# SCoulY/MuSCLe

Hardware: AMD Instinct MI355X
Metric: images/sec (whole node), MCL EfficientNet-B7 448x448 bs=32/GPU (higher is better)
Workload: dtype f32; 1 GPU; train_mcl.py loop body, step-A (epoch-4 gates: focal+softmargin+pairwise+ER+IMC, one backward, one Adam step), MuSCLe(efficientnet-b7, last_pooling=False, 21 classes), random-init weights; per_gpu_batch=32, global_batch=32, image=448x448, parallelism=single, optimizer=Adam(lr=1e-4, wd=5e-5) fused, launch=eager, weight-gradient GEMMs on a second stream

## Files before the change

### include/muscle_hip.h

```cpp
#ifndef MUSCLE_HIP_H
#define MUSCLE_HIP_H

#ifdef __cplusplus
extern "C" {
#endif

int mx_version(void);
int mx_abi_hash(void);
const char* mx_last_error(void);


int mx_pw_fwd_parts(int M, int N, int K);
int mx_pw_fwd(const float* A, int a_mode, const float* a_scale, const float* a_shift, const float* a_gate,
              int rows_per_sample, const float* W, float* C, int M, int K, int N, int lda, int ldc,
              const float* bias, const float* residual, int relu, float* stats, void* stream);

int mx_set_gemm_mode(int mode);
int mx_get_gemm_mode(void);
int mx_set_wgrad_kernel(int kernel, int groups);
int mx_get_wgrad_kernel(void);
int mx_gemm_uses_split(int kind, int M, int N, int K);

long mx_pw_planes_bytes(int N, int K);
int mx_pw_planes_tiles(int N, int K);
int mx_pw_planes_batch(const long* table, int n, int total_tiles, void* stream);
int mx_pw_fwd_uses_planes(int M, int K, int N);
int mx_pw_fwd_planes(const float* A, const void* Wplanes, float* C, int M, int K, int N, int lda, int ldc,
                     const float* bias, const float* residual, int relu, float* stats, void* stream);

int mx_transpose(const float* src, float* dst, int rows, int cols, void* stream);
int mx_transpose_batch(const long* table, int n, int total_tiles, void* stream);

int mx_pw_dgrad(const float* G, const float* W, float* dX, int M, int K, int N, int ldg, int ldx,
                const float* residual, void* stream);

int mx_pw_dgrad_bnbwd(const float* G, const float* X, const float* coef, const float* Wt, float* dX, float* dZ, int M, int K, int N,
                      int ldg, int ldx, const float* residual, void* stream);

int mx_pw_fwd_act_uses_planes(int M, int K, int N);
int mx_pw_fwd_planes_act(const float* A, const float* scale, const float* shift, const float* gate, int rows_per_sample,
                         const void* Wplanes, float* C, int M, int K, int N, int lda, int ldc, float* stats, void* stream);

int mx_pw_dgrad_bnbwd_planes(const float* G, const float* X, const float* coef, const void* WtPlanes, float* dX, int M, int K, int N,
// ... 30 lines not shown
int mx_colreduce_parts(long rows, int C);
int mx_colstats(const float* X, long rows, int C, float* part, void* stream);

int mx_bn_finalize(const float* part, int P, int C, double count, const float* gamma, const float* beta, float* running_mean,
                   float* running_var, float momentum, float eps, int training, float* scale, float* shift,
                   float* mean, float* rstd, double* acc , void* stream);

int mx_fold_block(const float* We, const float* g0, const float* b0, const float* m0, const float* v0, float eps0,
                  const float* g1, const float* b1, const float* m1, const float* v1, float eps1,
                  const float* Wp, const float* g2, const float* b2, const float* m2, const float* v2, float eps2,
                  int Cin, int Cexp, int Cout, float* We_f, float* be, float* s1, float* t1, float* Wp_f, float* bp, void* stream);

int mx_bn_apply(const float* P, const float* scale, const float* shift, const float* row_scale, const float* residual,
                const float* gate, float* out, long rows, int C, int rows_per_sample, int act, void* stream);

int mx_bn_bwd_reduce(const float* G, const float* X, const float* row_scale, const float* gate, const float* gate_add,
                     const float* act_scale, const float* act_shift, long rows, int C, int rows_per_sample,
                     float* part, void* stream);

int mx_bn_bwd_finalize(const float* part, int P, int C, double count, const float* gamma, const float* mean, const float* rstd,
                       int training, float* dgamma, float* dbeta, float* c1, float* c2, float* c3, double* acc,
                       void* stream);

int mx_bn_bwd_apply(const float* G, const float* X, const float* row_scale, const float* gate, const float* gate_add,
                    const float* act_scale, const float* act_shift, const float* c1, const float* c2, const float* c3,
                    float* out, long rows, int C, int rows_per_sample, void* stream);

long mx_pool_ws(long rows, int C, int rows_per_sample, int planes);
int mx_pool_sum(const float* X, const float* G, const float* scale, const float* shift, int act, long rows, int C,
                int rows_per_sample, float* out, void* ws, long ws_bytes, void* stream);

int mx_se_bn1_pool(const float* dA, const float* X, const float* scale, const float* shift, long rows, int C, int rows_per_sample,
                   float* out5, void* ws, long ws_bytes, void* stream);
int mx_bn1_sums_finalize(const float* pooled5, const float* gate, const float* gh, const float* W1, float inv_hw, float* add,
                         int N, int C, int SQ, double count, const float* gamma, const float* mean, const float* rstd, int training,
                         float* dgamma, float* dbeta, float* c1, float* c2, float* c3, void* stream);


int mx_dwconv_fwd_parts(int N, int Ho, int Wo, int C, int S);
long mx_dwconv_fwd_ws(int N, int Ho, int Wo, int C, int S);
int mx_dwconv_fwd(const float* X, const float* scale, const float* shift, const float* W, float* Y, float* stats,
// ... 175 lines not shown
```

### muscle_amd/csrc/bn.hip

```cpp
#include "common.h"

struct ColGeom {
  int rows, C, c4;
  int tcols;
  int rpp;
  int rows_per_block;
  int rps;
};

static ColGeom col_geom(long rows, int C, int rps, long rows_limit ,
                        int groups = 1 , int planes = 1) {
  ColGeom g;
  g.rows = (int)rows; g.C = C; g.c4 = C / 4; g.rps = rps;
  {
    const int cand[] = {g.c4 <= 256 ? g.c4 : 256, 256, 192, 128, 96, 64, 48, 32};
    double best = -1.0;
    g.tcols = cand[0];
    for (int tc : cand) {
      if (tc > g.c4) continue;
      const double util = (double)g.c4 / (double)(cdiv(g.c4, tc) * tc) * (double)(256 / tc * tc) / 256.0;
      if (groups > 1 ? util > best - 1e-9 : util > best + 1e-9) { best = util; g.tcols = tc; }
    }
  }
  g.rpp = 256 / g.tcols;
// ... 482 lines not shown
  int dr, dc, dn, drem, c4n, rps;
  __device__ __forceinline__ RowWalk(long i0, long stride, int c4n_, int rps_) : c4n(c4n_), rps(rps_) {
    r = i0 / c4n; c4 = (int)(i0 - r * c4n);
    n = (int)(r / rps); rem = (int)(r - (long)n * rps);
    const long sr = stride / c4n;
    dr = (int)sr; dc = (int)(stride - sr * c4n);
    dn = dr / rps; drem = dr - dn * rps;
  }
  __device__ __forceinline__ void next() {
    c4 += dc; r += dr; n += dn; rem += drem;
    if (c4 >= c4n) { c4 -= c4n; ++r; ++rem; }
    if (rem >= rps) { rem -= rps; ++n; }
  }
};

__global__ __launch_bounds__(256) void bn_apply_kernel(const float* P, const float* sc, const float* sh, const float* rs,
                                                       const float* R, const float* gate, float* out, long total4, int C,
                                                       int rps, int act) {
  RowWalk w(blockIdx.x * 256L + threadIdx.x, (long)gridDim.x * 256, C / 4, rps);
  for (long i = blockIdx.x * 256L + threadIdx.x; i < total4; i += (long)gridDim.x * 256, w.next()) {
    const int c = w.c4 * 4;
    float4 v = ld4(P + i * 4);
    float4 a = ld4(sc + c), b = ld4(sh + c);
    v.x = a.x * v.x + b.x; v.y = a.y * v.y + b.y; v.z = a.z * v.z + b.z; v.w = a.w * v.w + b.w;
    if (act) { v.x = swishf_(v.x); v.y = swishf_(v.y); v.z = swishf_(v.z); v.w = swishf_(v.w); }
    if (gate) { float4 g = ld4(gate + (long)w.n * C + c); v.x *= g.x; v.y *= g.y; v.z *= g.z; v.w *= g.w; }
    if (rs) { float s = rs[w.n]; v.x *= s; v.y *= s; v.z *= s; v.w *= s; }
    if (R) { float4 q = ld4(R + i * 4); v.x += q.x; v.y += q.y; v.z += q.z; v.w += q.w; }
    st4(out + i * 4, v);
  }
}

__global__ __launch_bounds__(256) void bn_bwd_apply_kernel(GEff e, const float* c1, const float* c2, const float* c3,
                                                           float* out, long total4) {
  RowWalk w(blockIdx.x * 256L + threadIdx.x, (long)gridDim.x * 256, e.C / 4, e.rps);
  for (long i = blockIdx.x * 256L + threadIdx.x; i < total4; i += (long)gridDim.x * 256, w.next()) {
    const int c = w.c4 * 4;
    float4 g, x;
    e.get_n(w.r, w.n, c, g, x);
    float4 k1 = ld4(c1 + c), k2 = ld4(c2 + c), k3 = ld4(c3 + c);
    float4 o;
    o.x = k1.x * g.x + k2.x * x.x + k3.x; o.y = k1.y * g.y + k2.y * x.y + k3.y;
    o.z = k1.z * g.z + k2.z * x.z + k3.z; o.w = k1.w * g.w + k2.w * x.w + k3.w;
    st4(out + i * 4, o);
  }
}

static int grid_for(long total4) {
  static const long cap = getenv("MX_STREAM_BLOCKS") ? atol(getenv("MX_STREAM_BLOCKS")) : 4096;
  long b = (total4 + 255) / 256;
  return (int)(b < cap ? (b < 1 ? 1 : b) : cap);
}

struct FoldArgs {
  const float *We, *g0, *b0, *m0, *v0, *g1, *b1, *m1, *v1, *Wp, *g2, *b2, *m2, *v2;
  float eps0, eps1, eps2;
  int Cin, Cexp, Cout;
  float *We_f, *be, *s1, *t1, *Wp_f, *bp;
};
// ... 67 lines not shown
    MX_LAUNCH_CHECK();
    return MX_OK;
  }
  int slices = 0;
  if (training) slices = launch_parts_reduce(part, P, C, acc, (hipStream_t)stream);
  hipLaunchKernelGGL(bn_finalize_kernel, dim3(cdiv(C, 32)), dim3(256), 0, (hipStream_t)stream, acc, slices, C, count, gamma,
                     beta, running_mean, running_var, momentum, eps, training, scale, shift, mean, rstd);
  MX_LAUNCH_CHECK();
  return MX_OK;
}

int mx_bn_apply(const float* P, const float* scale, const float* shift, const float* row_scale, const float* residual,
                const float* gate, float* out, long rows, int C, int rows_per_sample, int act, void* stream) {
  MX_CHECK_ARG(P && scale && shift && out && rows > 0 && C % 4 == 0 && rows_per_sample > 0, "bn_apply: bad args");
  long total4 = rows * (C / 4);
  hipLaunchKernelGGL(bn_apply_kernel, dim3(grid_for(total4)), dim3(256), 0, (hipStream_t)stream, P, scale, shift,
                     row_scale, residual, gate, out, total4, C, rows_per_sample, act);
  MX_LAUNCH_CHECK();
  return MX_OK;
}

int mx_bn_bwd_reduce(const float* G, const float* X, const float* row_scale, const float* gate, const float* gate_add,
                     const float* act_scale, const float* act_shift, long rows, int C, int rows_per_sample,
                     float* part, void* stream) {
  MX_CHECK_ARG(G && X && part && rows > 0 && C % 4 == 0 && rows_per_sample > 0, "bn_bwd_reduce: bad args");
  MX_CHECK_ARG((gate == nullptr) == (gate_add == nullptr), "bn_bwd_reduce: gate and gate_add come together");
  MX_CHECK_ARG((act_scale == nullptr) == (act_shift == nullptr), "bn_bwd_reduce: act scale/shift come together");
  FBwdReduce f{GEff{G, X, row_scale, gate, gate_add, act_scale, act_shift, C, rows_per_sample}};
  launch_colreduce<FBwdReduce, 2, false, float>(f, rows, C, rows_per_sample, part, part, (hipStream_t)stream);
  MX_LAUNCH_CHECK();
  return MX_OK;
}
// ... 9 lines not shown
    return MX_OK;
  }
  const int slices = launch_parts_reduce(part, P, C, acc, (hipStream_t)stream);
  hipLaunchKernelGGL(bn_bwd_finalize_kernel, dim3(cdiv(C, 32)), dim3(256), 0, (hipStream_t)stream, acc, slices, C, count, gamma,
                     mean, rstd, training, dgamma, dbeta, c1, c2, c3);
  MX_LAUNCH_CHECK();
  return MX_OK;
}

int mx_bn_bwd_apply(const float* G, const float* X, const float* row_scale, const float* gate, const float* gate_add,
                    const float* act_scale, const float* act_shift, const float* c1, const float* c2, const float* c3,
                    float* out, long rows, int C, int rows_per_sample, void* stream) {
  MX_CHECK_ARG(G && X && out && c1 && c2 && c3 && rows > 0 && C % 4 == 0 && rows_per_sample > 0, "bn_bwd_apply: bad args");
  GEff e{G, X, row_scale, gate, gate_add, act_scale, act_shift, C, rows_per_sample};
  long total4 = rows * (C / 4);
  hipLaunchKernelGGL(bn_bwd_apply_kernel, dim3(grid_for(total4)), dim3(256), 0, (hipStream_t)stream, e, c1, c2, c3, out,
                     total4);
  MX_LAUNCH_CHECK();
  return MX_OK;
}

long mx_pool_ws(long rows, int C, int rows_per_sample, int planes) {
  if (rows <= 0 || C <= 0 || C % 4 || rows_per_sample <= 0 || rows % rows_per_sample || (planes != 1 && planes != 5)) return MX_EARG;
  return pool_ws_bytes(rows, C, rows_per_sample, planes);
}

int mx_se_bn1_pool(const float* dA, const float* X, const float* scale, const float* shift, long rows, int C, int rows_per_sample,
                   float* out5, void* ws, long ws_bytes, void* stream) {
  MX_CHECK_ARG(dA && X && scale && shift && out5 && rows > 0 && C % 4 == 0 && rows_per_sample > 0 && rows % rows_per_sample == 0,
               "se_bn1_pool: bad args");
  const int N = (int)(rows / rows_per_sample);
  dim3 grid;
// ... 41 lines not shown
```

### muscle_amd/csrc/common.h

```cpp
#pragma once
#include <hip/hip_runtime.h>
#include <stdint.h>

#define MX_OK 0
#define MX_EARG (-1)

extern "C" const char* mx_last_error(void);
void mx_set_error(const char* fmt, ...);

#define MX_CHECK_ARG(cond, ...)            \
  do {                                     \
    if (!(cond)) {                         \
      mx_set_error(__VA_ARGS__);           \
      return MX_EARG;                      \
    }                                      \
  } while (0)

#define MX_LAUNCH_CHECK()                                     \
  do {                                                        \
    hipError_t e__ = hipGetLastError();                       \
    if (e__ != hipSuccess) {                                  \
      mx_set_error("launch failed: %s", hipGetErrorString(e__)); \
      return (int)e__;                                        \
    }                                                         \
// ... 126 lines not shown
  for (int i = 1; i < 8; ++i) { s0 += sh[i * 32 + cl]; s1 += sh[256 + i * 32 + cl]; }
  bn_bwd_finalize_one(c, s0, s1, b.count, b.gamma, b.mean, b.rstd, b.training, b.dgamma, b.dbeta, b.c1, b.c2, b.c3);
}

__device__ __forceinline__ float4 ld4(const float* p) { return *reinterpret_cast<const float4*>(p); }
__device__ __forceinline__ void st4(float* p, float4 v) { *reinterpret_cast<float4*>(p) = v; }

struct MxOperand {
  const float* p;
  const float* c1;
  const float* c2;
  const float* rowp;
  int mode;
  int rps;
};
enum { MX_PLAIN = 0, MX_BNACT = 1, MX_AFFINE = 2, MX_BNBWD = 3 };

__device__ __forceinline__ float4 mx_apply(const MxOperand& o, float4 v, long r, int c, int cols) {
  if (o.mode == MX_PLAIN) return v;
  float4 a = ld4(o.c1 + c), b = ld4(o.c2 + c);
  v.x = a.x * v.x + b.x; v.y = a.y * v.y + b.y; v.z = a.z * v.z + b.z; v.w = a.w * v.w + b.w;
  if (o.mode == MX_AFFINE) return v;
  v.x = swishf_(v.x); v.y = swishf_(v.y); v.z = swishf_(v.z); v.w = swishf_(v.w);
  if (o.rowp) {
    float4 g = ld4(o.rowp + (r / o.rps) * (long)cols + c);
    v.x *= g.x; v.y *= g.y; v.z *= g.z; v.w *= g.w;
  }
  return v;
}
```

### muscle_amd/csrc/gemm.hip

```cpp
#include "common.h"
#include <type_traits>
#include <stdlib.h>

typedef float f32x16 __attribute__((ext_vector_type(16)));
typedef float f32x4 __attribute__((ext_vector_type(4)));

struct GemmArgs {
  MxOperand a, b;
  float* c;
  int M, N, K;
  int lda, ldb, ldc;
  long sa, sb, sc;
  const float* bias;
  const float* residual;
  int relu;
  float* stats;
  int ksplit;
  int xcd_nt;
  int mt, zt;
  unsigned long long* stamps;
  float* a_out;
  float* ws;
};

// ... 568 lines not shown
    for (int st = 0; st < 4; ++st)
#pragma unroll
      for (int i = 0; i < TM; ++i)
#pragma unroll
        for (int j = 0; j < TN; ++j)
          acc[i][j] = __builtin_amdgcn_mfma_f32_16x16x4f32(bv[j][st], av[i][st], acc[i][j], 0, 0, 0);
    __syncthreads();
  }
  MX_GEMM_STAMP(g, 2);
  nt_epilogue<WM, WN, TM, TN>(g, C, tile_m, m0, n0, acc, smem, tid);
  MX_GEMM_STAMP(g, 3);
}

typedef __bf16 bf16x8 __attribute__((ext_vector_type(8)));

static __device__ __forceinline__ void split3_pair(float x0, float x1, unsigned& h, unsigned& m, unsigned& l) {
  const unsigned u0 = __float_as_uint(x0) & 0xffff0000u, u1 = __float_as_uint(x1) & 0xffff0000u;
  const float r0 = x0 - __uint_as_float(u0), r1 = x1 - __uint_as_float(u1);
  const unsigned v0 = __float_as_uint(r0) & 0xffff0000u, v1 = __float_as_uint(r1) & 0xffff0000u;
  const float s0 = r0 - __uint_as_float(v0), s1 = r1 - __uint_as_float(v1);
  h = __builtin_amdgcn_perm(u1, u0, 0x07060302u);
  m = __builtin_amdgcn_perm(v1, v0, 0x07060302u);
  l = __builtin_amdgcn_perm(__float_as_uint(s1), __float_as_uint(s0), 0x07060302u);
}

template <int AMODE, int NJ>
__global__ __launch_bounds__(256, NJ == 4 ? 2 : 3) void gemm_nt_split_kernel(GemmArgs g) {
  constexpr int BM = 128, BN = 64 * NJ, WN = 2, WNC = 32 * NJ;
  constexpr int PA_ = 128 * 32, PB_ = BN * 32;
  constexpr int STAGE = 3 * PA_ + 3 * PB_;
  constexpr int PS = WNC + 4;
  constexpr int SMEM = (2 * STAGE > 4 * 32 * PS * 4 + 2 * 2 * BN * 4) ? 2 * STAGE : 4 * 32 * PS * 4 + 2 * 2 * BN * 4;
  __shared__ __attribute__((aligned(16))) unsigned char smem[SMEM];
  const int tid = threadIdx.x, lane = tid & 63, wave = tid >> 6;
  const int l31 = lane & 31, hf = lane >> 5;
  const int wm = wave / WN, wn = wave % WN;
  int tile_m = blockIdx.x, tile_n = blockIdx.y;
  if (g.xcd_nt > 0) {
    const int L = blockIdx.x, xcd = L & 7, j = L >> 3;
// ... 257 lines not shown
    const int chunk = blockIdx.x / per_chunk, L = blockIdx.x % per_chunk, xcd = L & 7, j = L >> 3;
    tile_n = chunk * g.xcd_nt + j % g.xcd_nt;
    tile_m = (j / g.xcd_nt) * 8 + xcd;
    if (tile_m >= g.mt || tile_n >= g.zt) return;
  }
  const int m0 = tile_m * BM, n0 = tile_n * BN;
  const long zb = blockIdx.z;
  const float* A = g.a.p + zb * g.sa;
  const unsigned char* WP = reinterpret_cast<const unsigned char*>(g.b.p);
  float* C = g.c + zb * g.sc;
  const int nk = (g.K + 31) >> 5;
  const bool ktail = (g.K & 31) != 0;
  const long npad64 = (long)g.ldb * 64;

  const float* ap[2];
#pragma unroll
  for (int i = 0; i < 2; ++i) {
    const int gr = min(m0 + 32 * wave + 16 * i + l15, g.M - 1);
    ap[i] = A + (long)gr * g.lda + 4 * q;
  }
  const unsigned char* wsrc[WPW];
  int wdst[WPW];
#pragma unroll
  for (int i = 0; i < WPW; ++i) {
    const int pw = wave + 4 * i, p = pw / (BN / 16), rp = pw % (BN / 16);
    wsrc[i] = WP + ((long)p * g.ldb + n0 + 16 * rp) * 64 + lane * 16;
    wdst[i] = p * W_PLANE + rp * 1024;
  }
  auto issue_w = [&](int kt) {
    unsigned char* st = smem + (kt & 1) * STAGE;
#pragma unroll
    for (int i = 0; i < WPW; ++i)
      if (WPIECES % 4 == 0 || wave + 4 * i < WPIECES) glds16(wsrc[i] + 3 * npad64 * kt, st + wdst[i]);
  };
  f32x4 raw[2][2];
  f32x4 rawx[(AMODE == MX_BNBWD || AMODE == MX_BNACT) ? 2 : 1][2], cf[AMODE == MX_BNBWD ? 3 : AMODE == MX_BNACT ? 2 : 1][2];
  const long xoff = AMODE == MX_BNBWD ? (g.a.rowp + zb * g.sa) - A : 0;
  const float* gp[AMODE == MX_BNACT ? 2 : 1];
  if (AMODE == MX_BNACT) {
#pragma unroll
    for (int i = 0; i < 2; ++i) {
      const int gr = min(m0 + 32 * wave + 16 * i + l15, g.M - 1);
      gp[AMODE == MX_BNACT ? i : 0] = g.a.rowp + (long)(gr / g.a.rps) * g.K + 4 * q;
    }
  }
  auto load_a = [&](int kt) {
    const bool half = AMODE != MX_BNBWD && ktail && kt == nk - 1;
#pragma unroll
    for (int i = 0; i < 2; ++i) {
      raw[i][0] = *reinterpret_cast<const f32x4*>(ap[i] + 32 * kt);
      raw[i][1] = half ? f32x4{0.f, 0.f, 0.f, 0.f} : *reinterpret_cast<const f32x4*>(ap[i] + 32 * kt + 16);
      if (AMODE == MX_BNBWD) {
        rawx[AMODE == MX_BNBWD ? i : 0][0] = *reinterpret_cast<const f32x4*>(ap[i] + xoff + 32 * kt);
        rawx[AMODE == MX_BNBWD ? i : 0][1] = *reinterpret_cast<const f32x4*>(ap[i] + xoff + 32 * kt + 16);
      }
      if (AMODE == MX_BNACT) {
        rawx[AMODE == MX_BNACT ? i : 0][0] = *reinterpret_cast<const f32x4*>(gp[AMODE == MX_BNACT ? i : 0] + 32 * kt);
        rawx[AMODE == MX_BNACT ? i : 0][1] = *reinterpret_cast<const f32x4*>(gp[AMODE == MX_BNACT ? i : 0] + 32 * kt + 16);
      }
    }
    if (AMODE == MX_BNACT) {
// ... 15 lines not shown
#pragma unroll
  for (int i = 0; i < 2; ++i)
#pragma unroll
    for (int j = 0; j < TN; ++j) acc[i][j] = f32x4{0.f, 0.f, 0.f, 0.f};
  const int woff = l15 * 64 + ((q ^ swz_w(l15)) << 4);

  MX_GEMM_STAMP(g, 0);
  issue_w(0);
  load_a(0);
  MX_GEMM_STAMP(g, 1);
  for (int kt = 0; kt < nk; ++kt) {
    asm volatile("s_waitcnt vmcnt(0)" ::: "memory");
    bf16x8 af[2][3];
#pragma unroll
    for (int i = 0; i < 2; ++i) {
      if (AMODE == MX_BNBWD) {
#pragma unroll
        for (int u = 0; u < 2; ++u)
#pragma unroll
          for (int e = 0; e < 4; ++e)
            raw[i][u][e] = cf[0][u][e] * raw[i][u][e] + (cf[AMODE == MX_BNBWD ? 1 : 0][u][e] * rawx[AMODE == MX_BNBWD ? i : 0][u][e] +
                                                         cf[AMODE == MX_BNBWD ? 2 : 0][u][e]);
      }
      if (AMODE == MX_BNACT) {
#pragma unroll
        for (int u = 0; u < 2; ++u)
#pragma unroll
          for (int e = 0; e < 4; ++e)
            raw[i][u][e] = swishf_(cf[0][u][e] * raw[i][u][e] + cf[AMODE == MX_BNACT ? 1 : 0][u][e]) * rawx[AMODE == MX_BNACT ? i : 0][u][e];
      }
// ... 80 lines not shown
static void launch_nt_split3_t(const GemmArgs& g, int batch, hipStream_t st) {
  constexpr int BN = 16 * TN;
  const int mt = cdiv(g.M, 128), nt = cdiv(g.N, BN);
  GemmArgs a = g;
  a.mt = mt;
  a.xcd_nt = 0;
  dim3 grid(mt, nt, batch);
  if (nt >= 2 && mt >= 64) {
    const int chunks = nt <= 16 ? 1 : cdiv(nt, g_split3_xcd_chunk);
    a.xcd_nt = cdiv(nt, chunks); a.zt = nt;
    grid = dim3(chunks * 8 * cdiv(mt, 8) * a.xcd_nt, 1, batch);
  }
  if (g.a.mode == MX_BNBWD) hipLaunchKernelGGL((gemm_nt_split3_kernel<TN, MX_BNBWD>), grid, dim3(256), 0, st, a);
  else if (g.a.mode == MX_BNACT) {
    if constexpr (TN <= 6) hipLaunchKernelGGL((gemm_nt_split3_kernel<TN, MX_BNACT>), grid, dim3(256), 0, st, a);
  } else hipLaunchKernelGGL((gemm_nt_split3_kernel<TN, MX_PLAIN>), grid, dim3(256), 0, st, a);
}

static int g_split_nj = getenv("MX_GEMM_SPLIT_NJ") ? atoi(getenv("MX_GEMM_SPLIT_NJ")) : 0;
static void launch_nt_split3(const GemmArgs& g, int batch, hipStream_t st) {
  auto cost = [&](int bn, double eff) {
    const double per_cu = (double)cdiv(g.M, 128) * cdiv(g.N, bn) * batch / 256.0;
    return (per_cu + 0.5) * bn / eff;
  };
  const long wide_tiles = (long)cdiv(g.M, 128) * cdiv(g.N, 128) * batch;
  int bn = 128;
  if (g_split_nj >= 16) bn = g_split_nj;
  else if (g_split_nj == 1 || (g_split_nj != 2 && wide_tiles <= 300)) bn = 64;
  else if (g_split_nj != 2) {
    const bool shortk = g.K <= 512;
    const double e64 = shortk ? 0.90 : 0.85, e80 = shortk ? 0.97 : 0.90, e96 = shortk ? 1.03 : 0.94, e112 = 0.97;
// ... 209 lines not shown
  hipLaunchKernelGGL(split_planes_kernel, dim3(total_tiles), dim3(256), 0, (hipStream_t)stream, table, n);
  MX_LAUNCH_CHECK();
  return MX_OK;
}

int mx_pw_fwd_uses_planes(int M, int K, int N) {
  static const int on = getenv("MX_SPLIT2") ? atoi(getenv("MX_SPLIT2")) : 1;
  static const int early = getenv("MX_SPLIT3_EARLY") ? atoi(getenv("MX_SPLIT3_EARLY")) : 1;
  static const int tail = getenv("MX_SPLIT3_KTAIL") ? atoi(getenv("MX_SPLIT3_KTAIL")) : 1;
  if (!on || M <= 0 || K % 16) return 0;
  if (K % 32) return (g_gemm_mode != 0 && tail && K >= 48 && N >= 96) ? 1 : 0;
  if (nt_uses_split(N, K)) return 1;
  return (g_gemm_mode == 1 && early && K >= 192 && N >= 48) ? 1 : 0;
}

int mx_pw_fwd_planes(const float* A, const void* Wplanes, float* C, int M, int K, int N, int lda, int ldc,
                     const float* bias, const float* residual, int relu, float* stats, void* stream) {
  MX_CHECK_ARG(A && Wplanes && C, "pw_fwd_planes: null pointer");
  MX_CHECK_ARG(M > 0 && N > 0 && K > 0 && K % 16 == 0, "pw_fwd_planes: bad extents M=%d N=%d K=%d (K must be a multiple of 16)", M, N, K);
  MX_CHECK_ARG(lda % 4 == 0 && lda >= K && ldc >= N, "pw_fwd_planes: bad leading dimensions lda=%d ldc=%d", lda, ldc);
  MX_CHECK_ARG((((uintptr_t)A | (uintptr_t)Wplanes | (uintptr_t)C) & 15) == 0, "pw_fwd_planes: pointers must be 16-byte aligned");
  GemmArgs g{};
  g.a = MxOperand{A, nullptr, nullptr, nullptr, MX_PLAIN, 1};
  g.b = MxOperand{reinterpret_cast<const float*>(Wplanes), nullptr, nullptr, nullptr, MX_PLAIN, 1};
  g.c = C; g.M = M; g.N = N; g.K = K; g.lda = lda; g.ldb = (N + 127) & ~127; g.ldc = ldc;
  g.bias = bias; g.residual = residual; g.relu = relu; g.stats = stats;
  g.stamps = mx_gemm_stamps;
  launch_nt_split3(g, 1, (hipStream_t)stream);
  MX_LAUNCH_CHECK();
  return MX_OK;
}

int mx_pw_fwd_act_uses_planes(int M, int K, int N) {
  static const int on = getenv("MX_SPLIT3_ACT") ? atoi(getenv("MX_SPLIT3_ACT")) : 1;
  static const int split2 = getenv("MX_SPLIT2") ? atoi(getenv("MX_SPLIT2")) : 1;
  return (on && split2 && g_gemm_mode != 0 && M >= 65536 && K % 32 == 0 && K >= 192 && N >= 48 && N <= 128) ? 1 : 0;
}

// ... 123 lines not shown
```

### muscle_amd/engine.py

```python
from __future__ import annotations

import functools
import os

from dataclasses import dataclass, field
from typing import Dict, List, Optional

import torch

from . import ops
from .arch import BlockCfg, NetCfg
from .ops import BNState


@dataclass
class BlockTape:
    cfg: BlockCfg
    H: int
    W: int
    Ho: int
    Wo: int
    x: torch.Tensor
    x_st: Optional[BNState]
    e_raw: Optional[torch.Tensor] = None
# ... 184 lines not shown
    tape.stem_raw = raw.view(N, H0, W0, C0)
    tape.stem_bn = ops.bn_finalize(stats, N * H0 * W0, backbone._bn0, training)

    drop_scales: Dict[int, torch.Tensor] = {}
    if training and drop_u is None:
        idx = [b.index for b in cfg.blocks if b.skip and b.drop_rate]
        if idx:
            rates = tuple(1.0 - cfg.blocks[i].drop_rate for i in idx)
            key = (rates, str(dev))
            if key not in _keep_cache:
                _keep_cache[key] = torch.tensor(rates, dtype=torch.float32).to(dev).view(-1, 1)
            keep = _keep_cache[key]
            rs = torch.floor(keep + torch.rand(len(idx), N, device=dev)) / keep
            drop_scales = {i: rs[j] for j, i in enumerate(idx)}
    x, x_st, h, w = tape.stem_raw, tape.stem_bn, H0, W0
    fold = None
    if not training and not save and EVAL_FOLD:
        fold = getattr(backbone, "_eval_fold", None)
        if fold is not None and fold["fingerprint"] != fold_fingerprint(backbone, cfg):
            fold = backbone._eval_fold = fold_eval_bn(backbone, cfg)
        elif fold is None:
            fold = fold_eval_bn(backbone, cfg)
    for b in cfg.blocks:
        m = _blk(backbone, b.index)
        ho, wo = b.out_size(h), b.out_size(w)
        t = BlockTape(cfg=b, H=h, W=w, Ho=ho, Wo=wo, x=x, x_st=x_st)
        if fold is not None:
            t.out = _block_forward_eval(m, b, fold[b.index], (fold["one"], fold["zero"]), x, x_st, N, h, w, ho, wo)
            t.x = None
            tape.blocks.append(t)
            if b.index == 0:
                tape.cols = tape.stem_raw = None
            if len(tape.blocks) >= 2 and tape.blocks[-2].cfg.index not in cfg.taps:
                tape.blocks[-2].out = None
            x, x_st, h, w = t.out, None, ho, wo
            continue
        M, Mo = N * h * w, N * ho * wo
        if b.expand:
            assert x_st is None
            st0 = None
            t.e_raw = ops.pw_fwd(x.view(M, b.cin), m._expand_conv.weight.view(b.cexp, b.cin), b.cexp, want_stats=training,
                                 planes=tape.wp.get(id(m._expand_conv.weight)))
            if training:
                t.e_raw, st0 = t.e_raw
            t.e_raw = t.e_raw.view(N, h, w, b.cexp)
            t.bn0 = ops.bn_finalize(st0, M, m._bn0, training)
            dw_in, dw_st = t.e_raw, t.bn0
        else:
            dw_in, dw_st = x, x_st
        st1 = None
        t.d_raw = ops.dwconv_fwd(dw_in, m._depthwise_conv.weight, b.kernel, b.stride, b.pad_lo, ho, wo, st=dw_st,
                                 want_stats=training)
        if training:
            t.d_raw, st1 = t.d_raw
        t.bn1 = ops.bn_finalize(st1, Mo, m._bn1, training)
        d2 = t.d_raw.view(Mo, b.cexp)
        pooled = ops.pool_sum(d2, ho * wo, st=t.bn1, act=True)
# ... 9 lines not shown
                                 a_scale=t.bn1.scale, a_shift=t.bn1.shift, a_gate=t.gate, rows_per_sample=ho * wo,
                                 want_stats=training, planes=tape.wp.get(id(m._project_conv.weight)))
        if training:
            t.p_raw, st2 = t.p_raw
        t.bn2 = ops.bn_finalize(st2, Mo, m._bn2, training)
        if b.skip and training and b.drop_rate:
            if drop_u is not None:
                keep = 1.0 - b.drop_rate
                t.row_scale = torch.floor(keep + drop_u[b.index].to(dev, torch.float32)) / keep
            else:
                t.row_scale = drop_scales[b.index]
        res = None
        if b.skip:
            assert x_st is None
            res = x.view(M, b.cin)
        t.out = ops.bn_apply(t.p_raw, t.bn2, row_scale=t.row_scale, residual=res, rows_per_sample=ho * wo).view(N, ho, wo, b.cout)
        tape.blocks.append(t)
        x, x_st, h, w = t.out, None, ho, wo
        if not save:
            t.x = t.e_raw = t.d_raw = t.p_raw = t.a = None
            if b.index == 0:
                tape.cols = tape.stem_raw = None
            if len(tape.blocks) >= 2 and tape.blocks[-2].cfg.index not in cfg.taps:
                tape.blocks[-2].out = None
    ops.flush_batch_counters()
    return tape


class GradSink:

    def __init__(self):
        self.bufs: Dict[int, torch.Tensor] = {}

    def of(self, p: torch.nn.Parameter) -> torch.Tensor:
        g = self.bufs.get(id(p))
        if g is None:
            g = torch.zeros_like(p, memory_format=torch.contiguous_format)
            self.bufs[id(p)] = g
        return g


FUSED_DW_BACKWARD = True
FOLD_BN0_APPLY = os.environ.get("MUSCLE_FOLD_BN0", "0") == "1"
FOLD_BN0_BOTH = os.environ.get("MUSCLE_FOLD_BN0_BOTH", "0") == "1"
FOLD_BN0_EARLY = os.environ.get("MUSCLE_FOLD_BN0_EARLY", "1") == "1"
FOLD_BN0_WGRAD = os.environ.get("MUSCLE_FOLD_BN0_WGRAD", "0") == "1"
WGRAD_SIDE_STREAM = os.environ.get("MUSCLE_WGRAD_STREAM", "1") == "1"
_side_streams: Dict[tuple, "torch.cuda.Stream"] = {}


def _masked_stream(device, n_cus: int):
    import ctypes
    hip = ctypes.CDLL("libamdhip64.so")
    total = torch.cuda.get_device_properties(device).multi_processor_count
    n_cus = max(1, min(int(n_cus), total))
    words = (total + 31) // 32
    mask = (ctypes.c_uint32 * words)()
# ... 97 lines not shown
    N, training = tape.N, tape.training
    g_out: Optional[torch.Tensor] = None
    lane = _WgradLane(tape.blocks[0].out.device)
    if tape.wt_event is not None:
        torch.cuda.current_stream().wait_event(tape.wt_event)
    for t in reversed(tape.blocks):
        b, m = t.cfg, _blk(backbone, t.cfg.index)
        tg = tap_grads.get(b.index)
        if tg is not None:
            g_out = tg if g_out is None else g_out + tg
        if g_out is None:
            continue
        M, Mo = N * t.H * t.W, N * t.Ho * t.Wo
        hw = t.Ho * t.Wo
        g2 = g_out.reshape(Mo, b.cout)
        dp = ops.bn_backward(g2, t.p_raw, m._bn2, t.bn2, sink.of(m._bn2.weight), sink.of(m._bn2.bias), training,
                             row_scale=t.row_scale, rows_per_sample=hw)
        d2 = t.d_raw.view(Mo, b.cexp)
        if t.a is not None:
            lane.wgrad(dp, t.a, sink.of(m._project_conv.weight).view(b.cout, b.cexp))
            t.a = None
        else:
            lane.wgrad(dp, d2, sink.of(m._project_conv.weight).view(b.cout, b.cexp), x_mode=ops.BNACT, x_scale=t.bn1.scale,
                       x_shift=t.bn1.shift, x_gate=t.gate, rows_per_sample=hw)
        ga = ops.pw_dgrad(dp, m._project_conv.weight.view(b.cout, b.cexp), b.cexp, wt=tape.wt.get(id(m._project_conv.weight)),
                          planes=tape.wtp.get(id(m._project_conv.weight)))
        lane.flush()
        del dp
        pooled5 = ops.se_bn1_pool(ga, d2, t.bn1, hw)
        W2 = m._se_expand.weight.view(b.cexp, b.se)
        if SE_PARAMS_ASIDE:
            gh = ops.se_bwd_gh(pooled5[0], t.gate, t.h, W2)
            lane.defer(functools.partial(ops.se_bwd_params, pooled5[0], t.gate, t.s, t.h, gh,
                                         sink.of(m._se_reduce.weight).view(b.se, b.cexp), sink.of(m._se_reduce.bias),
                                         sink.of(m._se_expand.weight).view(b.cexp, b.se), sink.of(m._se_expand.bias)),
                       pooled5, t.gate, t.s, t.h, gh)
        else:
            gh = ops.se_bwd(pooled5[0], t.gate, t.s, t.h, W2,
                            sink.of(m._se_reduce.weight).view(b.se, b.cexp), sink.of(m._se_reduce.bias),
                            sink.of(m._se_expand.weight).view(b.cexp, b.se), sink.of(m._se_expand.bias))
        c1, add = ops.bn1_coeffs(pooled5, t.gate, gh, m._se_reduce.weight.view(b.se, b.cexp), 1.0 / hw, Mo, m._bn1, t.bn1,
                                 sink.of(m._bn1.weight), sink.of(m._bn1.bias), training)
        dw_in, dw_st = (t.e_raw, t.bn0) if b.expand else (t.x, t.x_st)
# ... 70 lines not shown
```

### muscle_amd/ops.py

```python
from __future__ import annotations

import os
from typing import NamedTuple, Optional

import torch

from ._lib import call, lib, ptr, stream

PLAIN, BNACT, AFFINE = 0, 1, 2


class BNState(NamedTuple):
    scale: torch.Tensor
    shift: torch.Tensor
    mean: torch.Tensor
    rstd: torch.Tensor


def _f32(*shape, device):
    return torch.empty(shape, dtype=torch.float32, device=device)


_scratch_bufs: dict = {}
_scratch_retired: list = []
# ... 30 lines not shown
    key = (get_gemm_mode(), M, K, N_out)
    r = _uses_planes.get(key)
    if r is None:
        r = _uses_planes[key] = bool(lib().mx_pw_fwd_uses_planes(M, K, N_out))
    return r


def _planes_act_take(M, K, N_out):
    key = ("act", get_gemm_mode(), M, K, N_out)
    r = _uses_planes.get(key)
    if r is None:
        r = _uses_planes[key] = bool(lib().mx_pw_fwd_act_uses_planes(M, K, N_out))
    return r


def pw_fwd(A, W, N_out, *, a_mode=PLAIN, a_scale=None, a_shift=None, a_gate=None, rows_per_sample=1,
           bias=None, residual=None, relu=False, want_stats=False, out=None, ldc=None, planes=None):
    M, K = A.shape
    ldc = ldc or N_out
    if out is None:
        out = _f32(M, ldc, device=A.device)
    stats = None
    if want_stats:
        stats = _f32(lib().mx_pw_fwd_parts(M, N_out, K), 2, N_out, device=A.device)
    if planes is not None and a_mode == PLAIN and _planes_take(M, K, N_out):
        call("mx_pw_fwd_planes", ptr(A), planes, ptr(out), M, K, N_out, A.stride(0), ldc, ptr(bias), ptr(residual), int(relu),
             ptr(stats), stream())
    elif (planes is not None and a_mode == BNACT and a_gate is not None and bias is None and residual is None and not relu
          and _planes_act_take(M, K, N_out)):
        call("mx_pw_fwd_planes_act", ptr(A), ptr(a_scale), ptr(a_shift), ptr(a_gate), rows_per_sample, planes, ptr(out), M, K, N_out,
             A.stride(0), ldc, ptr(stats), stream())
    else:
        call("mx_pw_fwd", ptr(A), a_mode, ptr(a_scale), ptr(a_shift), ptr(a_gate), rows_per_sample, ptr(W), ptr(out),
             M, K, N_out, A.stride(0), ldc, ptr(bias), ptr(residual), int(relu), ptr(stats), stream())
    return (out, stats) if want_stats else out


def set_gemm_mode(mode: int):
    call("mx_set_gemm_mode", int(mode))

# ... 85 lines not shown
    def run_backward(self):
        wt = self.t.run()
        return wt, self.bwd.run()


def transpose(W):
    rows, cols = W.shape
    out = _f32(cols, rows, device=W.device)
    call("mx_transpose", ptr(W), ptr(out), rows, cols, stream())
    return out


DGRAD_AS_FORWARD = True


def pw_dgrad(G, W, N_in, *, residual=None, out=None, wt=None, planes=None):
    M, K = G.shape
    if out is None:
        out = _f32(M, N_in, device=G.device)
    if DGRAD_AS_FORWARD and K % 4 == 0:
        if planes is not None and _planes_take(M, K, N_in):
            call("mx_pw_fwd_planes", ptr(G), planes, ptr(out), M, K, N_in, G.stride(0), N_in, None, ptr(residual), 0, None, stream())
            return out
        call("mx_pw_fwd", ptr(G), PLAIN, None, None, None, 1, ptr(wt if wt is not None else transpose(W)), ptr(out), M, K, N_in, G.stride(0), N_in,
             None, ptr(residual), 0, None, stream())
        return out
    call("mx_pw_dgrad", ptr(G), ptr(W), ptr(out), M, K, N_in, G.stride(0), N_in, ptr(residual), stream())
    return out


def pw_dgrad_bnbwd(G, X, coef, W, N_in, *, residual=None, wt=None):
    M, K = G.shape
    out = _f32(M, N_in, device=G.device)
    dz = torch.empty_like(G)
    call("mx_pw_dgrad_bnbwd", ptr(G), ptr(X), ptr(coef), ptr(wt if wt is not None else transpose(W)), ptr(out), ptr(dz), M, K, N_in,
         G.stride(0), N_in, ptr(residual), stream())
# ... 156 lines not shown
        if t is not None:
            _scratch_retired.append(t)
        t = _acc_bufs[key] = torch.empty(max(n, 128 * 4096), dtype=torch.float64, device=dev)
    return t.data_ptr()


_nbt_pending: list = []


def flush_batch_counters():
    if _nbt_pending:
        torch._foreach_add_(_nbt_pending, 1)
        _nbt_pending.clear()


def bn_apply(P2d, st: BNState, *, row_scale=None, residual=None, gate=None, rows_per_sample=1, act=False, out=None):
    rows, C = P2d.shape
    if out is None:
        out = torch.empty_like(P2d)
    call("mx_bn_apply", ptr(P2d), ptr(st.scale), ptr(st.shift), ptr(row_scale), ptr(residual), ptr(gate), ptr(out), rows, C,
         rows_per_sample, int(act), stream())
    return out


def bn_backward(G2d, X2d, bn: torch.nn.BatchNorm2d, st: BNState, dgamma, dbeta, training: bool, *, row_scale=None,
                gate=None, gate_add=None, act: Optional[BNState] = None, rows_per_sample=1, out=None):
    rows, C = X2d.shape
    P = lib().mx_colreduce_parts(rows, C)
    sums = _f32(P, 2, C, device=X2d.device)
    a_sc = act.scale if act is not None else None
    a_sh = act.shift if act is not None else None
    call("mx_bn_bwd_reduce", ptr(G2d), ptr(X2d), ptr(row_scale), ptr(gate), ptr(gate_add), ptr(a_sc), ptr(a_sh), rows, C,
         rows_per_sample, ptr(sums), stream())
    c = _f32(3, C, device=X2d.device)
    call("mx_bn_bwd_finalize", ptr(sums), P, C, float(rows), ptr(bn.weight), ptr(st.mean), ptr(st.rstd), int(training),
         ptr(dgamma), ptr(dbeta), ptr(c[0]), ptr(c[1]), ptr(c[2]),
         _acc_scratch(X2d.device, 128 * C), stream())
    if out is None:
        out = torch.empty_like(X2d)
    call("mx_bn_bwd_apply", ptr(G2d), ptr(X2d), ptr(row_scale), ptr(gate), ptr(gate_add), ptr(a_sc), ptr(a_sh),
         ptr(c[0]), ptr(c[1]), ptr(c[2]), ptr(out), rows, C, rows_per_sample, stream())
    return out


def bn_backward_from_coeffs(G2d, X2d, st: BNState, c, *, gate, gate_add, rows_per_sample, out):
    rows, C = X2d.shape
    cb, cs = c.data_ptr(), 4 * C
    call("mx_bn_bwd_apply", ptr(G2d), ptr(X2d), None, ptr(gate), ptr(gate_add), ptr(st.scale), ptr(st.shift),
         cb, cb + cs, cb + 2 * cs, ptr(out), rows, C, rows_per_sample, stream())
    return out


def bn_bwd_coeffs(part, rows, bn, st: BNState, dgamma, dbeta, training: bool):
    P, _, C = part.shape
# ... 271 lines not shown
```

Baseline: 339.7 images/sec.

## Emit pre-split bf16x3 A-operand planes from BN apply kernels for plane GEMMs

The forward bn_apply and backward bn_bwd_apply kernels now optionally write, alongside the fp32 output, a pre-split three-plane bf16 image of the activation in the tiled layout the split3 GEMM consumes. The next block's expand conv and the project-conv dgrad bind that image so the GEMM loads A planes directly instead of re-reading fp32 A and splitting it per tile. This removes the split arithmetic and some layout work from the GEMM inner loop. In exchange the BN kernels write 1.5x more bytes, extra scratch buffers are allocated, and plane binding goes through thread-local state.

```diff
diff --git a/include/muscle_hip.h b/include/muscle_hip.h
--- a/include/muscle_hip.h
+++ b/include/muscle_hip.h
@@ -27,6 +27,9 @@
 int mx_pw_fwd_uses_planes(int M, int K, int N);
 int mx_pw_fwd_planes(const float* A, const void* Wplanes, float* C, int M, int K, int N, int lda, int ldc,
                      const float* bias, const float* residual, int relu, float* stats, void* stream);
+
+long mx_a_planes_bytes(long M, int K);
+int mx_pw_fwd_planes_bind_a(const void* Aplanes);
 
 int mx_transpose(const float* src, float* dst, int rows, int cols, void* stream);
 int mx_transpose_batch(const long* table, int n, int total_tiles, void* stream);
@@ -87,6 +90,9 @@
 int mx_bn_apply(const float* P, const float* scale, const float* shift, const float* row_scale, const float* residual,
                 const float* gate, float* out, long rows, int C, int rows_per_sample, int act, void* stream);
 
+int mx_bn_apply_planes(const float* P, const float* scale, const float* shift, const float* row_scale, const float* residual,
+                       const float* gate, float* out, long rows, int C, int rows_per_sample, int act, void* planes, void* stream);
+
 int mx_bn_bwd_reduce(const float* G, const float* X, const float* row_scale, const float* gate, const float* gate_add,
                      const float* act_scale, const float* act_shift, long rows, int C, int rows_per_sample,
                      float* part, void* stream);
@@ -98,6 +104,10 @@
 int mx_bn_bwd_apply(const float* G, const float* X, const float* row_scale, const float* gate, const float* gate_add,
                     const float* act_scale, const float* act_shift, const float* c1, const float* c2, const float* c3,
                     float* out, long rows, int C, int rows_per_sample, void* stream);
+
+int mx_bn_bwd_apply_planes(const float* G, const float* X, const float* row_scale, const float* gate, const float* gate_add,
+                           const float* act_scale, const float* act_shift, const float* c1, const float* c2, const float* c3,
+                           float* out, long rows, int C, int rows_per_sample, void* planes, void* stream);
 
 long mx_pool_ws(long rows, int C, int rows_per_sample, int planes);
 int mx_pool_sum(const float* X, const float* G, const float* scale, const float* shift, int act, long rows, int C,
diff --git a/muscle_amd/csrc/bn.hip b/muscle_amd/csrc/bn.hip
--- a/muscle_amd/csrc/bn.hip
+++ b/muscle_amd/csrc/bn.hip
@@ -520,9 +520,21 @@
   }
 };
 
+static __device__ __forceinline__ void st_a_planes(unsigned char* img, long r, int c4, int nk, float4 v) {
+  unsigned h0, m0, l0, h1, m1, l1;
+  split3_pair(v.x, v.y, h0, m0, l0);
+  split3_pair(v.z, v.w, h1, m1, l1);
+  const int j = c4 & 7;
+  unsigned char* d = img + a_planes_off(r, c4 >> 3, j & 3, nk) + (j >> 2) * 8;
+  *reinterpret_cast<uint2*>(d) = make_uint2(h0, h1);
+  *reinterpret_cast<uint2*>(d + 1024) = make_uint2(m0, m1);
+  *reinterpret_cast<uint2*>(d + 2048) = make_uint2(l0, l1);
+}
+
+template <bool PLANES>
 __global__ __launch_bounds__(256) void bn_apply_kernel(const float* P, const float* sc, const float* sh, const float* rs,
                                                        const float* R, const float* gate, float* out, long total4, int C,
-                                                       int rps, int act) {
+                                                       int rps, int act, unsigned char* img) {
   RowWalk w(blockIdx.x * 256L + threadIdx.x, (long)gridDim.x * 256, C / 4, rps);
   for (long i = blockIdx.x * 256L + threadIdx.x; i < total4; i += (long)gridDim.x * 256, w.next()) {
     const int c = w.c4 * 4;
@@ -534,11 +546,13 @@
     if (rs) { float s = rs[w.n]; v.x *= s; v.y *= s; v.z *= s; v.w *= s; }
     if (R) { float4 q = ld4(R + i * 4); v.x += q.x; v.y += q.y; v.z += q.z; v.w += q.w; }
     st4(out + i * 4, v);
-  }
-}
-
+    if (PLANES) st_a_planes(img, w.r, w.c4, C >> 5, v);
+  }
+}
+
+template <bool PLANES>
 __global__ __launch_bounds__(256) void bn_bwd_apply_kernel(GEff e, const float* c1, const float* c2, const float* c3,
-                                                           float* out, long total4) {
+                                                           float* out, long total4, unsigned char* img) {
   RowWalk w(blockIdx.x * 256L + threadIdx.x, (long)gridDim.x * 256, e.C / 4, e.rps);
   for (long i = blockIdx.x * 256L + threadIdx.x; i < total4; i += (long)gridDim.x * 256, w.next()) {
     const int c = w.c4 * 4;
@@ -549,6 +563,7 @@
     o.x = k1.x * g.x + k2.x * x.x + k3.x; o.y = k1.y * g.y + k2.y * x.y + k3.y;
     o.z = k1.z * g.z + k2.z * x.z + k3.z; o.w = k1.w * g.w + k2.w * x.w + k3.w;
     st4(out + i * 4, o);
+    if (PLANES) st_a_planes(img, w.r, w.c4, e.C >> 5, o);
   }
 }
 
@@ -646,8 +661,20 @@
                 const float* gate, float* out, long rows, int C, int rows_per_sample, int act, void* stream) {
   MX_CHECK_ARG(P && scale && shift && out && rows > 0 && C % 4 == 0 && rows_per_sample > 0, "bn_apply: bad args");
   long total4 = rows * (C / 4);
-  hipLaunchKernelGGL(bn_apply_kernel, dim3(grid_for(total4)), dim3(256), 0, (hipStream_t)stream, P, scale, shift,
-                     row_scale, residual, gate, out, total4, C, rows_per_sample, act);
+  hipLaunchKernelGGL(bn_apply_kernel<false>, dim3(grid_for(total4)), dim3(256), 0, (hipStream_t)stream, P, scale, shift,
+                     row_scale, residual, gate, out, total4, C, rows_per_sample, act, (unsigned char*)nullptr);
+  MX_LAUNCH_CHECK();
+  return MX_OK;
+}
+
+int mx_bn_apply_planes(const float* P, const float* scale, const float* shift, const float* row_scale, const float* residual,
+                       const float* gate, float* out, long rows, int C, int rows_per_sample, int act, void* planes, void* stream) {
+  MX_CHECK_ARG(P && scale && shift && out && planes && rows > 0 && C > 0 && C % 32 == 0 && rows_per_sample > 0,
+               "bn_apply_planes: bad args (C = %d must be a multiple of 32)", C);
+  MX_CHECK_ARG(((uintptr_t)planes & 15) == 0, "bn_apply_planes: the image must be 16-byte aligned");
+  long total4 = rows * (C / 4);
+  hipLaunchKernelGGL(bn_apply_kernel<true>, dim3(grid_for(total4)), dim3(256), 0, (hipStream_t)stream, P, scale, shift,
+                     row_scale, residual, gate, out, total4, C, rows_per_sample, act, (unsigned char*)planes);
   MX_LAUNCH_CHECK();
   return MX_OK;
 }
@@ -687,8 +714,22 @@
   MX_CHECK_ARG(G && X && out && c1 && c2 && c3 && rows > 0 && C % 4 == 0 && rows_per_sample > 0, "bn_bwd_apply: bad args");
   GEff e{G, X, row_scale, gate, gate_add, act_scale, act_shift, C, rows_per_sample};
   long total4 = rows * (C / 4);
-  hipLaunchKernelGGL(bn_bwd_apply_kernel, dim3(grid_for(total4)), dim3(256), 0, (hipStream_t)stream, e, c1, c2, c3, out,
-                     total4);
+  hipLaunchKernelGGL(bn_bwd_apply_kernel<false>, dim3(grid_for(total4)), dim3(256), 0, (hipStream_t)stream, e, c1, c2, c3, out,
+                     total4, (unsigned char*)nullptr);
+  MX_LAUNCH_CHECK();
+  return MX_OK;
+}
+
+int mx_bn_bwd_apply_planes(const float* G, const float* X, const float* row_scale, const float* gate, const float* gate_add,
+                           const float* act_scale, const float* act_shift, const float* c1, const float* c2, const float* c3,
+                           float* out, long rows, int C, int rows_per_sample, void* planes, void* stream) {
+  MX_CHECK_ARG(G && X && out && c1 && c2 && c3 && planes && rows > 0 && C > 0 && C % 32 == 0 && rows_per_sample > 0,
+               "bn_bwd_apply_planes: bad args (C = %d must be a multiple of 32)", C);
+  MX_CHECK_ARG(((uintptr_t)planes & 15) == 0, "bn_bwd_apply_planes: the image must be 16-byte aligned");
+  GEff e{G, X, row_scale, gate, gate_add, act_scale, act_shift, C, rows_per_sample};
+  long total4 = rows * (C / 4);
+  hipLaunchKernelGGL(bn_bwd_apply_kernel<true>, dim3(grid_for(total4)), dim3(256), 0, (hipStream_t)stream, e, c1, c2, c3, out,
+                     total4, (unsigned char*)planes);
   MX_LAUNCH_CHECK();
   return MX_OK;
 }
diff --git a/muscle_amd/csrc/common.h b/muscle_amd/csrc/common.h
--- a/muscle_amd/csrc/common.h
+++ b/muscle_amd/csrc/common.h
@@ -164,7 +164,21 @@
   int mode;
   int rps;
 };
-enum { MX_PLAIN = 0, MX_BNACT = 1, MX_AFFINE = 2, MX_BNBWD = 3 };
+enum { MX_PLAIN = 0, MX_BNACT = 1, MX_AFFINE = 2, MX_BNBWD = 3, MX_APLANES = 4 };
+
+__device__ __forceinline__ void split3_pair(float x0, float x1, unsigned& h, unsigned& m, unsigned& l) {
+  const unsigned u0 = __float_as_uint(x0) & 0xffff0000u, u1 = __float_as_uint(x1) & 0xffff0000u;
+  const float r0 = x0 - __uint_as_float(u0), r1 = x1 - __uint_as_float(u1);
+  const unsigned v0 = __float_as_uint(r0) & 0xffff0000u, v1 = __float_as_uint(r1) & 0xffff0000u;
+  const float s0 = r0 - __uint_as_float(v0), s1 = r1 - __uint_as_float(v1);
+  h = __builtin_amdgcn_perm(u1, u0, 0x07060302u);
+  m = __builtin_amdgcn_perm(v1, v0, 0x07060302u);
+  l = __builtin_amdgcn_perm(__float_as_uint(s1), __float_as_uint(s0), 0x07060302u);
+}
+
+__device__ __forceinline__ long a_planes_off(long r, int kt, int q, int nk) {
+  return (((r >> 4) * nk + kt) * 3) * 1024 + (r & 15) * 64 + q * 16;
+}
 
 __device__ __forceinline__ float4 mx_apply(const MxOperand& o, float4 v, long r, int c, int cols) {
   if (o.mode == MX_PLAIN) return v;
diff --git a/muscle_amd/csrc/gemm.hip b/muscle_amd/csrc/gemm.hip
--- a/muscle_amd/csrc/gemm.hip
+++ b/muscle_amd/csrc/gemm.hip
@@ -606,15 +606,6 @@
 
 typedef __bf16 bf16x8 __attribute__((ext_vector_type(8)));
 
-static __device__ __forceinline__ void split3_pair(float x0, float x1, unsigned& h, unsigned& m, unsigned& l) {
-  const unsigned u0 = __float_as_uint(x0) & 0xffff0000u, u1 = __float_as_uint(x1) & 0xffff0000u;
-  const float r0 = x0 - __uint_as_float(u0), r1 = x1 - __uint_as_float(u1);
-  const unsigned v0 = __float_as_uint(r0) & 0xffff0000u, v1 = __float_as_uint(r1) & 0xffff0000u;
-  const float s0 = r0 - __uint_as_float(v0), s1 = r1 - __uint_as_float(v1);
-  h = __builtin_amdgcn_perm(u1, u0, 0x07060302u);
-  m = __builtin_amdgcn_perm(v1, v0, 0x07060302u);
-  l = __builtin_amdgcn_perm(__float_as_uint(s1), __float_as_uint(s0), 0x07060302u);
-}
 
 template <int AMODE, int NJ>
 __global__ __launch_bounds__(256, NJ == 4 ? 2 : 3) void gemm_nt_split_kernel(GemmArgs g) {
@@ -902,10 +893,12 @@
   const long npad64 = (long)g.ldb * 64;
 
   const float* ap[2];
+  const unsigned char* app[AMODE == MX_APLANES ? 2 : 1];
 #pragma unroll
   for (int i = 0; i < 2; ++i) {
     const int gr = min(m0 + 32 * wave + 16 * i + l15, g.M - 1);
     ap[i] = A + (long)gr * g.lda + 4 * q;
+    if (AMODE == MX_APLANES) app[AMODE == MX_APLANES ? i : 0] = reinterpret_cast<const unsigned char*>(g.a.p) + a_planes_off(gr, 0, q, nk);
   }
   const unsigned char* wsrc[WPW];
   int wdst[WPW];
@@ -932,7 +925,16 @@
       gp[AMODE == MX_BNACT ? i : 0] = g.a.rowp + (long)(gr / g.a.rps) * g.K + 4 * q;
     }
   }
+  bf16x8 afn[AMODE == MX_APLANES ? 2 : 1][3];
   auto load_a = [&](int kt) {
+    if (AMODE == MX_APLANES) {
+#pragma unroll
+      for (int i = 0; i < 2; ++i)
+#pragma unroll
+        for (int p = 0; p < 3; ++p)
+          afn[AMODE == MX_APLANES ? i : 0][p] = *reinterpret_cast<const bf16x8*>(app[AMODE == MX_APLANES ? i : 0] + (long)(3 * kt + p) * 1024);
+      return;
+    }
     const bool half = AMODE != MX_BNBWD && ktail && kt == nk - 1;
 #pragma unroll
     for (int i = 0; i < 2; ++i) {
@@ -978,6 +980,11 @@
     bf16x8 af[2][3];
 #pragma unroll
     for (int i = 0; i < 2; ++i) {
+      if (AMODE == MX_APLANES) {
+#pragma unroll
+        for (int p = 0; p < 3; ++p) af[i][p] = afn[AMODE == MX_APLANES ? i : 0][p];
+        continue;
+      }
       if (AMODE == MX_BNBWD) {
 #pragma unroll
         for (int u = 0; u < 2; ++u)
@@ -1088,7 +1095,8 @@
   if (g.a.mode == MX_BNBWD) hipLaunchKernelGGL((gemm_nt_split3_kernel<TN, MX_BNBWD>), grid, dim3(256), 0, st, a);
   else if (g.a.mode == MX_BNACT) {
     if constexpr (TN <= 6) hipLaunchKernelGGL((gemm_nt_split3_kernel<TN, MX_BNACT>), grid, dim3(256), 0, st, a);
-  } else hipLaunchKernelGGL((gemm_nt_split3_kernel<TN, MX_PLAIN>), grid, dim3(256), 0, st, a);
+  } else if (g.a.mode == MX_APLANES) hipLaunchKernelGGL((gemm_nt_split3_kernel<TN, MX_APLANES>), grid, dim3(256), 0, st, a);
+  else hipLaunchKernelGGL((gemm_nt_split3_kernel<TN, MX_PLAIN>), grid, dim3(256), 0, st, a);
 }
 
 static int g_split_nj = getenv("MX_GEMM_SPLIT_NJ") ? atoi(getenv("MX_GEMM_SPLIT_NJ")) : 0;
@@ -1328,14 +1336,30 @@
   return (g_gemm_mode == 1 && early && K >= 192 && N >= 48) ? 1 : 0;
 }
 
+long mx_a_planes_bytes(long M, int K) {
+  if (M <= 0 || K <= 0 || K % 32) return MX_EARG;
+  return ((M + 15) & ~15L) * K * 6;
+}
+
+static thread_local const void* t_bound_a = nullptr;
+int mx_pw_fwd_planes_bind_a(const void* Aplanes) {
+  MX_CHECK_ARG(((uintptr_t)Aplanes & 15) == 0, "pw_fwd_planes_bind_a: the image must be 16-byte aligned");
+  t_bound_a = Aplanes;
+  return MX_OK;
+}
+
 int mx_pw_fwd_planes(const float* A, const void* Wplanes, float* C, int M, int K, int N, int lda, int ldc,
                      const float* bias, const float* residual, int relu, float* stats, void* stream) {
+  const void* Aplanes = t_bound_a;
+  t_bound_a = nullptr;
   MX_CHECK_ARG(A && Wplanes && C, "pw_fwd_planes: null pointer");
+  MX_CHECK_ARG(!Aplanes || K % 32 == 0, "pw_fwd_planes: an A-plane image needs K %% 32 == 0 (K=%d)", K);
   MX_CHECK_ARG(M > 0 && N > 0 && K > 0 && K % 16 == 0, "pw_fwd_planes: bad extents M=%d N=%d K=%d (K must be a multiple of 16)", M, N, K);
   MX_CHECK_ARG(lda % 4 == 0 && lda >= K && ldc >= N, "pw_fwd_planes: bad leading dimensions lda=%d ldc=%d", lda, ldc);
   MX_CHECK_ARG((((uintptr_t)A | (uintptr_t)Wplanes | (uintptr_t)C) & 15) == 0, "pw_fwd_planes: pointers must be 16-byte aligned");
   GemmArgs g{};
   g.a = MxOperand{A, nullptr, nullptr, nullptr, MX_PLAIN, 1};
+  if (Aplanes) g.a = MxOperand{reinterpret_cast<const float*>(Aplanes), nullptr, nullptr, nullptr, MX_APLANES, 1};
   g.b = MxOperand{reinterpret_cast<const float*>(Wplanes), nullptr, nullptr, nullptr, MX_PLAIN, 1};
   g.c = C; g.M = M; g.N = N; g.K = K; g.lda = lda; g.ldb = (N + 127) & ~127; g.ldc = ldc;
   g.bias = bias; g.residual = residual; g.relu = relu; g.stats = stats;
diff --git a/muscle_amd/engine.py b/muscle_amd/engine.py
--- a/muscle_amd/engine.py
+++ b/muscle_amd/engine.py
@@ -222,6 +222,7 @@
             rs = torch.floor(keep + torch.rand(len(idx), N, device=dev)) / keep
             drop_scales = {i: rs[j] for j, i in enumerate(idx)}
     x, x_st, h, w = tape.stem_raw, tape.stem_bn, H0, W0
+    x_planes = None
     fold = None
     if not training and not save and EVAL_FOLD:
         fold = getattr(backbone, "_eval_fold", None)
@@ -229,7 +230,7 @@
             fold = backbone._eval_fold = fold_eval_bn(backbone, cfg)
         elif fold is None:
             fold = fold_eval_bn(backbone, cfg)
-    for b in cfg.blocks:
+    for bi, b in enumerate(cfg.blocks):
         m = _blk(backbone, b.index)
         ho, wo = b.out_size(h), b.out_size(w)
         t = BlockTape(cfg=b, H=h, W=w, Ho=ho, Wo=wo, x=x, x_st=x_st)
@@ -248,7 +249,8 @@
             assert x_st is None
             st0 = None
             t.e_raw = ops.pw_fwd(x.view(M, b.cin), m._expand_conv.weight.view(b.cexp, b.cin), b.cexp, want_stats=training,
-                                 planes=tape.wp.get(id(m._expand_conv.weight)))
+                                 planes=tape.wp.get(id(m._expand_conv.weight)), a_planes=x_planes)
+            x_planes = None
             if training:
                 t.e_raw, st0 = t.e_raw
             t.e_raw = t.e_raw.view(N, h, w, b.cexp)
@@ -288,7 +290,13 @@
         if b.skip:
             assert x_st is None
             res = x.view(M, b.cin)
-        t.out = ops.bn_apply(t.p_raw, t.bn2, row_scale=t.row_scale, residual=res, rows_per_sample=ho * wo).view(N, ho, wo, b.cout)
+        nb = cfg.blocks[bi + 1] if bi + 1 < len(cfg.blocks) else None
+        want_planes = (A_PLANES and nb is not None and nb.expand and tape.wp.get(id(_blk(backbone, nb.index)._expand_conv.weight)) is not None
+                       and ops.a_planes_take(Mo, b.cout, nb.cexp))
+        t.out = ops.bn_apply(t.p_raw, t.bn2, row_scale=t.row_scale, residual=res, rows_per_sample=ho * wo, want_planes=want_planes)
+        if want_planes:
+            t.out, x_planes = t.out
+        t.out = t.out.view(N, ho, wo, b.cout)
         tape.blocks.append(t)
         x, x_st, h, w = t.out, None, ho, wo
         if not save:
@@ -315,6 +323,7 @@
 
 
 FUSED_DW_BACKWARD = True
+A_PLANES = os.environ.get("MUSCLE_A_PLANES", "1") != "0"
 FOLD_BN0_APPLY = os.environ.get("MUSCLE_FOLD_BN0", "0") == "1"
 FOLD_BN0_BOTH = os.environ.get("MUSCLE_FOLD_BN0_BOTH", "0") == "1"
 FOLD_BN0_EARLY = os.environ.get("MUSCLE_FOLD_BN0_EARLY", "1") == "1"
@@ -442,8 +451,11 @@
         M, Mo = N * t.H * t.W, N * t.Ho * t.Wo
         hw = t.Ho * t.Wo
         g2 = g_out.reshape(Mo, b.cout)
+        wtp_p = tape.wtp.get(id(m._project_conv.weight))
+        dp_planes = A_PLANES and wtp_p is not None and ops.DGRAD_AS_FORWARD and ops.a_planes_take(Mo, b.cout, b.cexp)
         dp = ops.bn_backward(g2, t.p_raw, m._bn2, t.bn2, sink.of(m._bn2.weight), sink.of(m._bn2.bias), training,
-                             row_scale=t.row_scale, rows_per_sample=hw)
+                             row_scale=t.row_scale, rows_per_sample=hw, want_planes=dp_planes)
+        dp, dp_planes = dp if dp_planes else (dp, None)
         d2 = t.d_raw.view(Mo, b.cexp)
         if t.a is not None:
             lane.wgrad(dp, t.a, sink.of(m._project_conv.weight).view(b.cout, b.cexp))
@@ -452,9 +464,9 @@
             lane.wgrad(dp, d2, sink.of(m._project_conv.weight).view(b.cout, b.cexp), x_mode=ops.BNACT, x_scale=t.bn1.scale,
                        x_shift=t.bn1.shift, x_gate=t.gate, rows_per_sample=hw)
         ga = ops.pw_dgrad(dp, m._project_conv.weight.view(b.cout, b.cexp), b.cexp, wt=tape.wt.get(id(m._project_conv.weight)),
-                          planes=tape.wtp.get(id(m._project_conv.weight)))
+                          planes=wtp_p, a_planes=dp_planes)
         lane.flush()
-        del dp
+        del dp, dp_planes
         pooled5 = ops.se_bn1_pool(ga, d2, t.bn1, hw)
         W2 = m._se_expand.weight.view(b.cexp, b.se)
         if SE_PARAMS_ASIDE:
diff --git a/muscle_amd/ops.py b/muscle_amd/ops.py
--- a/muscle_amd/ops.py
+++ b/muscle_amd/ops.py
@@ -68,8 +68,16 @@
     return r
 
 
+def a_planes_take(M, K, N_out):
+    return K % 32 == 0 and get_gemm_mode() != 0 and _planes_take(M, K, N_out)
+
+
+def a_planes_alloc(rows, C, device):
+    return torch.empty(lib().mx_a_planes_bytes(rows, C), dtype=torch.uint8, device=device)
+
+
 def pw_fwd(A, W, N_out, *, a_mode=PLAIN, a_scale=None, a_shift=None, a_gate=None, rows_per_sample=1,
-           bias=None, residual=None, relu=False, want_stats=False, out=None, ldc=None, planes=None):
+           bias=None, residual=None, relu=False, want_stats=False, out=None, ldc=None, planes=None, a_planes=None):
     M, K = A.shape
     ldc = ldc or N_out
     if out is None:
@@ -78,6 +86,8 @@
     if want_stats:
         stats = _f32(lib().mx_pw_fwd_parts(M, N_out, K), 2, N_out, device=A.device)
     if planes is not None and a_mode == PLAIN and _planes_take(M, K, N_out):
+        if a_planes is not None:
+            call("mx_pw_fwd_planes_bind_a", ptr(a_planes))
         call("mx_pw_fwd_planes", ptr(A), planes, ptr(out), M, K, N_out, A.stride(0), ldc, ptr(bias), ptr(residual), int(relu),
              ptr(stats), stream())
     elif (planes is not None and a_mode == BNACT and a_gate is not None and bias is None and residual is None and not relu
@@ -193,12 +203,14 @@
 DGRAD_AS_FORWARD = True
 
 
-def pw_dgrad(G, W, N_in, *, residual=None, out=None, wt=None, planes=None):
+def pw_dgrad(G, W, N_in, *, residual=None, out=None, wt=None, planes=None, a_planes=None):
     M, K = G.shape
     if out is None:
         out = _f32(M, N_in, device=G.device)
     if DGRAD_AS_FORWARD and K % 4 == 0:
         if planes is not None and _planes_take(M, K, N_in):
+            if a_planes is not None:
+                call("mx_pw_fwd_planes_bind_a", ptr(a_planes))
             call("mx_pw_fwd_planes", ptr(G), planes, ptr(out), M, K, N_in, G.stride(0), N_in, None, ptr(residual), 0, None, stream())
             return out
         call("mx_pw_fwd", ptr(G), PLAIN, None, None, None, 1, ptr(wt if wt is not None else transpose(W)), ptr(out), M, K, N_in, G.stride(0), N_in,
@@ -385,17 +397,22 @@
         _nbt_pending.clear()
 
 
-def bn_apply(P2d, st: BNState, *, row_scale=None, residual=None, gate=None, rows_per_sample=1, act=False, out=None):
+def bn_apply(P2d, st: BNState, *, row_scale=None, residual=None, gate=None, rows_per_sample=1, act=False, out=None, want_planes=False):
     rows, C = P2d.shape
     if out is None:
         out = torch.empty_like(P2d)
+    if want_planes:
+        img = a_planes_alloc(rows, C, P2d.device)
+        call("mx_bn_apply_planes", ptr(P2d), ptr(st.scale), ptr(st.shift), ptr(row_scale), ptr(residual), ptr(gate), ptr(out), rows, C,
+             rows_per_sample, int(act), ptr(img), stream())
+        return out, img
     call("mx_bn_apply", ptr(P2d), ptr(st.scale), ptr(st.shift), ptr(row_scale), ptr(residual), ptr(gate), ptr(out), rows, C,
          rows_per_sample, int(act), stream())
     return out
 
 
 def bn_backward(G2d, X2d, bn: torch.nn.BatchNorm2d, st: BNState, dgamma, dbeta, training: bool, *, row_scale=None,
-                gate=None, gate_add=None, act: Optional[BNState] = None, rows_per_sample=1, out=None):
+                gate=None, gate_add=None, act: Optional[BNState] = None, rows_per_sample=1, out=None, want_planes=False):
     rows, C = X2d.shape
     P = lib().mx_colreduce_parts(rows, C)
     sums = _f32(P, 2, C, device=X2d.device)
@@ -409,6 +426,11 @@
          _acc_scratch(X2d.device, 128 * C), stream())
     if out is None:
         out = torch.empty_like(X2d)
+    if want_planes:
+        img = a_planes_alloc(rows, C, X2d.device)
+        call("mx_bn_bwd_apply_planes", ptr(G2d), ptr(X2d), ptr(row_scale), ptr(gate), ptr(gate_add), ptr(a_sc), ptr(a_sh),
+             ptr(c[0]), ptr(c[1]), ptr(c[2]), ptr(out), rows, C, rows_per_sample, ptr(img), stream())
+        return out, img
     call("mx_bn_bwd_apply", ptr(G2d), ptr(X2d), ptr(row_scale), ptr(gate), ptr(gate_add), ptr(a_sc), ptr(a_sh),
          ptr(c[0]), ptr(c[1]), ptr(c[2]), ptr(out), rows, C, rows_per_sample, stream())
     return out
```

Result: no change. 337.8 images/sec (-0.5%).
